# Lightbrite88/Argon_Monte_Carlo

Hardware: AMD Instinct MI355X
Metric: particle-steps/sec (higher is better)
Workload: dtype f64; 1 GPU; cube_1e5; geometry=cube, n_particles=100000, n_per_gpu=100000, parallelism=single GPU

## Files before the change

### argon_monte_carlo_amd/csrc/amc_api.hip

```cpp
#include <memory>
#include <type_traits>

#include "amc_host.h"

int amc_fail(amc_ctx *c, int code, const char *fmt, ...)
{
    char buf[512];
    va_list ap;
    va_start(ap, fmt);
    vsnprintf(buf, sizeof buf, fmt, ap);
    va_end(ap);
    if (c) c->err = buf;
    return code;
}

static thread_local std::string g_create_err;

void amc_prof_begin(amc_ctx *c, int kclass)
{
    if (!c->profiling) return;
    if (c->ev_used == c->ev_pool.size()) {
        hipEvent_t a, b;
        (void)ctx_event(c, &a, hipEventDefault);
        (void)ctx_event(c, &b, hipEventDefault);
// ... 95 lines not shown
    }
    if (off > 0x7fff0000LL) return amc_fail(c, AMC_ERR_INVALID, "detection grid too large (%lld cells)", off);
    G.ncells = (int)off;
    AMC_HIP(c, dalloc(c, &c->d_lay, (size_t)3 * G.gz));
    AMC_HIP(c, hipMemcpy(c->d_lay, c->h_lay_lo.data(), sizeof(int) * G.gz, hipMemcpyHostToDevice));
    AMC_HIP(c, hipMemcpy(c->d_lay + G.gz, c->h_lay_n.data(), sizeof(int) * G.gz, hipMemcpyHostToDevice));
    AMC_HIP(c, hipMemcpy(c->d_lay + 2 * G.gz, c->h_lay_off.data(), sizeof(int) * G.gz, hipMemcpyHostToDevice));
    G.lay_lo = c->d_lay; G.lay_n = c->d_lay + G.gz; G.lay_off = c->d_lay + 2 * G.gz;
    return AMC_OK;
}

static bool env_set(const char *name) { return getenv(name) != nullptr; }
static bool env_nonzero(const char *name) { const char *e = getenv(name); return e && atoi(e) != 0; }
static int env_int(const char *name, int unset) { const char *e = getenv(name); return e ? atoi(e) : unset; }
static long long env_ll(const char *name, long long unset) { const char *e = getenv(name); return e ? atoll(e) : unset; }

static void read_env(amc_ctx *c)
{
    const char *sync = getenv("AMC_OVERLAP_SYNC");
    c->ovl_sync_values = sync && !strcmp(sync, "value");
    c->overlap_mode = env_int("AMC_OVERLAP", 0);
    c->overlap_split = env_nonzero("AMC_OVERLAP_SPLIT");
    c->cw_blocks_env = env_int("AMC_CW_BLOCKS", 0);
    c->ordered_always = env_nonzero("AMC_ORDERED_ALWAYS");
    c->od_max_n = env_ll("AMC_OD_MAX_N", c->od_max_n);
    c->od_ahead = std::min(std::max(env_int("AMC_OD_AHEAD", c->od_ahead), 1), 32);
    if (const int v = env_int("AMC_PLAN_SMALL", -1); v >= 0) c->plan_small = v;
    c->stream_bs = env_int("AMC_STREAM_BS", 256);
    c->detect_bs = env_int("AMC_DETECT_BS", 256);
    c->temp_unfused = env_set("AMC_TEMP_UNFUSED");
    c->temp_run_unfused = !AMC_TEMP_RUN_FUSED_DEFAULT;
    if (env_nonzero("AMC_TEMP_RUN_FUSED")) c->temp_run_unfused = false;
    if (env_nonzero("AMC_TEMP_RUN_UNFUSED")) c->temp_run_unfused = true;
    c->allpairs_max_n = env_ll("AMC_ALLPAIRS_MAX_N", 0);
    const int g = c->P.geometry;
    c->list_keep = env_int("AMC_LIST_KEEP", (g == AMC_GEOM_PORE || g == AMC_GEOM_PORE_ENERGISED) ? AMC_LIST_KEEP_DEFAULT_PORE : 0);
    c->max_hist_env = env_int("AMC_MAX_HIST", 0);
    c->debug_resolve = env_set("AMC_DEBUG_RESOLVE");
}

static int alloc_state(amc_ctx *c)
{
    const size_t n = std::max<size_t>((size_t)c->n, 1);
    double **st[] = {&c->S.x, &c->S.y, &c->S.z, &c->S.vx, &c->S.vy, &c->S.vz, &c->S.d, &c->S.dx, &c->S.dy, &c->S.dz,
                     &c->S.px, &c->S.py, &c->S.pz};
    const size_t per = ((sizeof(double) * n) + 255) & ~(size_t)255;
// ... 451 lines not shown
        for (int v : h) { sum += v; top = std::max<int64_t>(top, v); }
    }
    out[0] = c->keep_K >= 2 ? c->keep_K : 0; out[1] = c->keep_K >= 2 ? c->B.wave_cap : 0; out[2] = (int64_t)waves;
    out[3] = cycle ? T.lists_age : -1; out[4] = owner; out[5] = sum; out[6] = top; out[7] = T.full_builds;
    return AMC_OK;
}

int amc_owned_count(amc_ctx *c, int64_t *count)
{
    if (!c || !count) return AMC_ERR_INVALID;
    *count = (int64_t)c->owned.size();
    return AMC_OK;
}

int amc_kernel_times(amc_ctx *c, double *total_ms, int64_t *launches)
{
    if (!c) return AMC_ERR_INVALID;
    hipSetDevice(c->device);
    amc_prof_collect(c);
    if (c->d_dbg) {
        long long h[128];
        hipMemcpy(h, c->d_dbg, sizeof h, hipMemcpyDeviceToHost);
        const double n = h[11] > 0 ? (double)h[11] : 1.0;
        fprintf(stderr, "[amc k_resolve phases, us/launch] count-left %.1f claim %.1f | rounds: collect %.1f pairs %.1f clusters>=3: sort+load %.1f emulate %.1f | overlay %.1f validate %.1f commit %.1f | rounds %.2f cand %.1f complex-members %.2f launches %lld (idle hand-over only %lld) | body: labels in the work space %lld moved there %lld layers in LDS %lld rounds split %lld heads shared %lld sorted %lld pool global %lld sort global %lld later %lld clusters by a wave %lld by one lane %lld most complex members %lld\n",
                h[0] / n / 100.0, h[1] / n / 100.0, h[6] / n / 100.0, h[7] / n / 100.0, h[2] / n / 100.0, h[3] / n / 100.0, h[14] / n / 100.0, h[4] / n / 100.0, h[5] / n / 100.0,
                h[8] / n, h[9] / n, h[10] / n, h[11], h[12], h[32], h[33], h[34], h[35], h[36], h[37], h[38], h[39], h[40], h[41], h[42], h[43]);
        fprintf(stderr, "[amc host candidate count] %d (what the next launch plan is chosen from)\n", c->h_host_ncand ? (int)*c->h_host_ncand : -1);
        if (h[12] > 0)
            fprintf(stderr, "[amc k_resolve idle hand-over, us/launch] entry -> counts read %.2f, -> hand-over written %.2f, -> through the barrier %.2f (%lld launches)\n",
                    h[16] / (double)h[12] / 100.0, h[17] / (double)h[12] / 100.0, h[18] / (double)h[12] / 100.0, h[12]);
        {
            std::vector<long long> wv((size_t)128 * 512);
            hipMemcpy(wv.data(), c->d_dbg + 128, sizeof(long long) * wv.size(), hipMemcpyDeviceToHost);
            long long s[128] = {0}, longest = 0;
            for (int w = 0; w < 512; w++) {
                for (int e = 3; e < 128; e++) if (e != 4) s[e] += wv[(size_t)128 * w + e];
                longest = std::max(longest, wv[(size_t)128 * w + 4]);
            }
            const double nl = h[25] > 0 ? (double)h[25] : 1.0;
            static const char *cn[8] = {"pair", "3-cluster", "4+-cluster", "not owner", "pair+again", "3-cluster+again", "4+-cluster+again", "not owner+again"};
            static const char *pn[12] = {"graph", "walk", "reserve", "small: after emulate", "pair emulate | by the wave: emulate", "publish", "grid probe", "first hop", "particles", "set-up", "overlay probe", "small: prepare"};
            fprintf(stderr, "[amc k_clusters_wide] working waves %lld in %lld launches; launch span (first working wave in -> last out) %.2f us, last out -> ordered workgroup in %.2f us, longest wave ever %.2f us\n",
                    s[3], h[25], h[27] / nl / 100.0, h[26] / nl / 100.0, longest / 100.0);
            fprintf(stderr, "[three-particle path of lane 0] %lld times, %lld continued from the pair's hit; loads + slots %.2f us, emulation %.2f us\n", s[5], s[6],
                    s[7] / (double)std::max<long long>(1, s[5]) / 100.0, s[124] / (double)std::max<long long>(1, s[5]) / 100.0);
            fprintf(stderr, "[pair-wave lifetimes, 2.5 us buckets]");
            for (int k = 0; k < 8; k++) fprintf(stderr, " %lld", s[24 + k]);
            fprintf(stderr, "\n");
            for (int k = 0; k < 8; k++) {
                if (!s[16 + k]) continue;
                fprintf(stderr, "[amc k_clusters_wide %-16s %7lld waves, %5.1f us]", cn[k], s[16 + k], s[8 + k] / (double)s[16 + k] / 100.0);
                for (int e = 0; e < 12; e++) fprintf(stderr, " %s %.2f", pn[e], s[32 + 12 * k + e] / (double)s[16 + k] / 100.0);
                fprintf(stderr, "\n");
            }
        }
    }
    for (int k = 0; k < AMC_K_COUNT; k++) {
        if (total_ms) total_ms[k] = c->k_ms[k];
        if (launches) launches[k] = c->k_launches[k];
    }
    return AMC_OK;
}

}
```

### argon_monte_carlo_amd/csrc/amc_clusters.hip

```cpp
#include <stdlib.h>

#define RS_WAVE_SYNC_LDS_ONLY 1
#include "amc_resolve_dev.h"

#define CW_MAXM 16
#define CW_MAXC 24
#define CW_ITEMS 192
#define CW_BLOCKS 512
#define CW_WPB 1

AMC_DEV int cw_adj_head(const amc_resolve_ws &W, unsigned int epoch, int p)
{
    const unsigned long long v = amc_g(W.adj_head)[p];
    return ((unsigned int)(v >> 32) == epoch) ? (int)(unsigned int)(v & 0xffffffffULL) : -1;
}

#define CW_ITERS 3
#define CW_PULLS 4

AMC_DEV void cw_init_slot(const amc_resolve_ws &W, int s, int p, int label, int gen, bool fresh = false)
{
    amc_g(W.slot_of)[p] = s; amc_g(W.sl_moved)[s] = 0;
    auto *m = amc_g((unsigned long long *)&W.sl_meta[s]);
    __hip_atomic_store(m + 0, ((unsigned long long)(unsigned int)label << 32) | (unsigned int)p, __ATOMIC_RELAXED, __HIP_MEMORY_SCOPE_AGENT);
// ... 5 lines not shown
{
    const auto *d = amc_g((const double *)&W.hist[h]);
    double4 r;
    r.x = __hip_atomic_load(d + 0, __ATOMIC_RELAXED, __HIP_MEMORY_SCOPE_AGENT);
    r.y = __hip_atomic_load(d + 1, __ATOMIC_RELAXED, __HIP_MEMORY_SCOPE_AGENT);
    r.z = __hip_atomic_load(d + 2, __ATOMIC_RELAXED, __HIP_MEMORY_SCOPE_AGENT);
    r.w = __hip_atomic_load(d + 3, __ATOMIC_RELAXED, __HIP_MEMORY_SCOPE_AGENT);
    return r;
}

struct cw_lds {
    int mem[64][CW_MAXM];
    int msl[64][CW_MAXM];
    int cnd[64][CW_MAXC];
    int pull[64][CW_PULLS], psl[64][CW_PULLS];
    int nm[64], nc[64], lab[64], npull[64];
    int it0[64];
    int used[64];
    int redo[64];
    int gen[64];
    cw_item item[CW_ITEMS];
    int next[CW_ITEMS];
    int nitems;
    int unv[64];
    double pool_d[10][CW_MAXM];
    int pool_tmp[CW_MAXM], pool_pidx[CW_MAXM], pool_slot[CW_MAXM];
    uint8_t pool_flag[CW_MAXM], pool_moved[CW_MAXM];
};

AMC_DEV void cw_probe_grid(const rs_args &A, rs_shared *wc, cw_lds &L, const cw_item &me, int cell, int s_off)
{
    const amc_resolve_ws &W = A.W;
    const int own = me.own, nm = L.nm[own], lab = L.lab[own];
    const double x = me.x, y = me.y, z = me.z;
    int q = amc_list_head(A.B, cell);
    while (q >= 0) {
        const amc_rec r = amc_g_load(&A.B.rec[q]);
        const int idx = amc_node_particle(A.B, q);
        q = amc_rec_next(r);
        double rx, ry, rz;
        amc_rec_pos(A.G, r, rx, ry, rz);
        const double ax = rx - x, ay = ry - y, az = rz - z;
        if (!(ax * ax + ay * ay + az * az < A.G.cr2_probe)) continue;
        bool mine = false;
        for (int m = 0; m < nm; m++) mine |= L.mem[own][m] == idx;
        if (mine) continue;
// ... 33 lines not shown
            if (t < 0 || t >= CW_ITEMS || L.item[t].h != h2) break;
            h2 = L.next[t];
        }
        return h2;
    };
    int h2 = skip_own(__hip_atomic_load(amc_g(W.ov_head) + cell, __ATOMIC_RELAXED, __HIP_MEMORY_SCOPE_AGENT));
    int guard = 0;
    while (h2 >= 0) {
        if (++guard > W.max_hist) { amc_g(wc)->ovf = 1; rs_raise(W); break; }
        const double4 o = cw_load_hist(W, h2);
        const int nx = __hip_atomic_load(amc_g(W.ov_next) + h2, __ATOMIC_RELAXED, __HIP_MEMORY_SCOPE_AGENT);
        h2 = skip_own(nx);
        const double ax = o.x - x, ay = o.y - y, az = o.z - z;
        if (!(ax * ax + ay * ay + az * az < cr2i)) continue;
        const int s2 = rs_hist_slot(o);
        bool mine = false;
        for (int m = 0; m < nm; m++) mine |= L.msl[own][m] == s2;
        if (mine) continue;
        if (rs_hist_gen(o) != __hip_atomic_load(amc_g((int *)&W.sl_meta[s2]) + 2, __ATOMIC_RELAXED, __HIP_MEMORY_SCOPE_AGENT)) continue;
        rs_add_edge(W, wc, me.p, -(s2 + 2));
    }
}

AMC_DEV int cw_prepare(const amc_resolve_ws &W, rs_shared *wc, cw_lds &L, int own, int h_off)
{
    int m = L.nm[own];
    const int lab = L.lab[own];
    const int np = L.npull[own] < CW_PULLS ? L.npull[own] : CW_PULLS;
    L.unv[own] = 0;
    for (int e = 0; e < np; e++) {
        const int v = L.pull[own][e], sv = L.psl[own][e];
        if (m == CW_MAXM) {
            cw_init_slot(W, sv, v, lab, 0);
            L.unv[own] = 2;
            continue;
        }
        int b = m - 1;
        while (b >= 0 && L.mem[own][b] > v) { L.mem[own][b + 1] = L.mem[own][b]; L.msl[own][b + 1] = L.msl[own][b]; b--; }
        L.mem[own][b + 1] = v; L.msl[own][b + 1] = sv;
        m++;
    }
    L.nm[own] = m; L.npull[own] = 0;
    L.used[own] = 0;
    L.it0[own] = -1;
    return m;
}
// ... 38 lines not shown
    int4 c4_first = make_int4(0, 0, -1, -1);
    unsigned long long mark_first = 0;
    if (lane < per && k_first < A_in_kernarg.W.max_cand) {
        c4_first = A_in_kernarg.W.cand4[k_first]; mark_first = A_in_kernarg.W.cand_mark[k_first];
    }
    int ncand = (int)__hip_atomic_load(&A_in_kernarg.O.cnt->cand_count, __ATOMIC_RELAXED, __HIP_MEMORY_SCOPE_AGENT);
    const int stalled = A_in_kernarg.od_stall ? *A_in_kernarg.od_stall : 0;
#pragma unroll
    for (int j = 0; j < ARG_TRIPS; j++) {
        const int i = (int)threadIdx.x + j * ARG_T;
        if (i < ARG_WORDS) ((int *)&s_args)[i] = arg_w[j];
    }
    __syncthreads();
    const rs_args &A = s_args;
    const amc_resolve_ws &W = A.W;
    rs_shared *wc = (rs_shared *)W.wctl;
    __shared__ cw_lds L_all[CW_WPB];
    cw_lds &L = L_all[threadIdx.x >> 6];
    if (stalled && A.od_tick > stalled) return;
    if (ncand > W.max_cand) ncand = W.max_cand;
    if (wave_id == 0 && lane == 0) {
        amc_g(wc)->active = 1; amc_g(wc)->ncand = ncand;
        if (A.od_done) *amc_g(A.od_done) = A.od_tick;
    }
    if (ncand == 0) return;
    const int s_off = 2 * ncand;
    const int h_off = 4 * ncand;
    const double cr2i = A.P.collision_range * A.P.collision_range * AMC_CR2_INFLATE;
    rs_work K;
    K.x = L.pool_d[0]; K.y = L.pool_d[1]; K.z = L.pool_d[2]; K.vx = L.pool_d[3]; K.vy = L.pool_d[4]; K.vz = L.pool_d[5];
    K.d = L.pool_d[6]; K.dx = L.pool_d[7]; K.dy = L.pool_d[8]; K.dz = L.pool_d[9];
    K.tmp = L.pool_tmp; K.pidx = L.pool_pidx; K.slot = L.pool_slot; K.flag = L.pool_flag; K.moved = L.pool_moved;

    long long t_last = t_enter__;
    long long t_acc[12] = {0, 0, 0, 0, 0, 0, 0, 0, 0, 0, 0, 0};
#define CW_STAMP(slot)                                                                     \
    do {                                                                                   \
        if (timed__) {                                                                     \
            const long long now__ = wall_clock64();                                        \
            t_acc[slot] += now__ - t_last;                                                 \
            t_last = now__;                                                                \
        }                                                                                  \
    } while (0)
    const bool timed__ = DBG && dbg__ && lane == 0 && wave_id * per < ncand;
    if (DBG && dbg__) { asm volatile("s_waitcnt vmcnt(0)" ::: "memory"); CW_STAMP(7); }
    int cat__ = 0;
    long long d_cont = 0, d_three = 0, d_t_load = 0, d_t_emu = 0;
    for (int k0 = wave_id * per; k0 < ncand; k0 += nwaves * per) {
        const int k = k0 + lane;
        const bool valid = lane < per && k < ncand;
        if (lane == 0) L.nitems = 0;
        int4 c4 = make_int4(0, 0, -1, -1);
        int head_i = -1, head_j = -1;
        amc_particle pre_j, pre_i;
        bool fh_ok = false;
        int fh_it0 = -1, fh_pj = -1, fh_pi = -1, fh_sj = -1, fh_si = -1;
        bool iso = false;
        int k2 = -1;
        int4 c4b = make_int4(0, 0, -1, -1);
        unsigned long long mkb = 0;
        if (valid) {
            c4 = (k == k_first) ? c4_first : amc_g_load(&W.cand4[k]);
            const unsigned long long mk = (k == k_first) ? mark_first : amc_g(W.cand_mark)[k];
            const bool marked = (unsigned int)(mk >> 32) == A.sweep_epoch;
            iso = c4.z < 0 && c4.w < 0 && !marked;
            if (c4.z < 0 && c4.w < 0 && marked) {
                const unsigned int succ = (unsigned int)(mk & 0xffffffffULL);
                if (succ != AMC_MARK_MULTI && (int)succ > k && (int)succ < ncand) k2 = (int)succ;
            }
            if (k2 >= 0) { c4b = amc_g_load(&W.cand4[k2]); mkb = amc_g(W.cand_mark)[k2]; }
// ... 172 lines not shown
                    for (int c = sub; c < 8; c += lpi) {
                        const int cell = amc_grid_box_cell<true>(A.G, it.x, it.y, it.z, A.G.cr_probe, c);
                        if (cell >= 0) cw_probe_grid(A, wc, L, it, cell, s_off);
                    }
                }
            }
            first_item = nit;
            CW_STAMP(6);
            if (!__ballot(L.redo[lane] != 0)) break;
            if (timed__ && L.redo[0]) cat__ |= 4;
            if (iter + 1 == CW_ITERS || L.nitems >= CW_ITEMS - 8) {
                if (L.redo[lane]) {
                    const int np = L.npull[lane] < CW_PULLS ? L.npull[lane] : CW_PULLS;
                    for (int e = 0; e < np; e++) cw_init_slot(W, L.psl[lane][e], L.pull[lane][e], L.lab[lane], 0);
                    rs_add_edge(W, wc, L.mem[lane][0], L.mem[lane][0]);
                    L.redo[lane] = 0;
                }
                break;
            }
        }
        rs_wave_sync();
        asm volatile("s_waitcnt vmcnt(0)" ::: "memory");
        const int nit = L.nitems < CW_ITEMS ? L.nitems : CW_ITEMS;
        for (int t0 = 0; t0 < nit; t0 += 64) {
            const int t = t0 + lane;
            if (t < nit) L.next[t] = -1;
            if (t < nit) {
                const cw_item it = L.item[t];
                if (!(it.pad & 1) && (it.pad >> 1) == L.gen[it.own]) {
                    int cx, cy, cz;
                    amc_grid_coords(A.G, it.x, it.y, it.z, cx, cy, cz);
                    const int cell = amc_grid_cell<true>(A.G, cx, cy, cz, nullptr);
                    int expected = -1;
                    for (;;) {
                        const int old = amc_atomic_cas(amc_g(W.ov_head) + cell, expected, it.h);
                        if (old == expected) break;
                        expected = old;
                        __hip_atomic_store(amc_g(W.ov_next) + it.h, old, __ATOMIC_RELAXED, __HIP_MEMORY_SCOPE_AGENT);
                        asm volatile("s_waitcnt vmcnt(0)" ::: "memory");
                    }
                    L.next[t] = expected;
                }
            }
        }
        asm volatile("s_waitcnt vmcnt(0)" ::: "memory");
        rs_wave_sync();
        CW_STAMP(5);
        {
            const int lpi = nit <= 8 ? 8 : (nit <= 16 ? 4 : (nit <= 32 ? 2 : 1));
            const int sub = lane % lpi;
            for (int t = lane / lpi; t < nit; t += 64 / lpi) {
                const cw_item it = L.item[t];
                if ((it.pad & 1) || (it.pad >> 1) != L.gen[it.own]) continue;
                for (int c = sub; c < 8; c += lpi) {
                    const int cell = amc_grid_box_cell<true>(A.G, it.x, it.y, it.z, A.G.cr_probe, c);
                    if (cell >= 0) cw_probe_overlay(A, wc, L, it, cell, cr2i, h_off);
                }
            }
        }
        rs_wave_sync();
        CW_STAMP(10);
    }
    if (timed__) {
        long long *R = dbg__ + 128 + 128 * (long long)wave_id;
        const long long t_exit = wall_clock64(), life = t_exit - t_enter__;
        R[0] = t_enter__; R[1] = t_exit; R[2] = A.sweep_epoch;
        R[3] += 1;
        if (life > R[4]) R[4] = life;
        R[5] += d_three; R[6] += d_cont; R[7] += d_t_load; R[124] += d_t_emu;
        R[8 + cat__] += life; R[16 + cat__] += 1;
        for (int e = 0; e < 12; e++) R[32 + 12 * cat__ + e] += t_acc[e];
        if (cat__ == 0) { int bk = (int)(life / 250); if (bk > 7) bk = 7; R[24 + bk] += 1; }
    }
}

int amc_clusters_wide_blocks(amc_ctx *c)
{
    const int nb_env = c->cw_blocks_env;
    if (nb_env > 0) return (nb_env + CW_WPB - 1) / CW_WPB * CW_WPB;
    return CW_BLOCKS;
}

hipError_t amc_launch_clusters_wide(amc_ctx *c, const rs_args &A)
{
    const int nb = amc_clusters_wide_blocks(c);
    const dim3 grid((nb + CW_WPB - 1) / CW_WPB), block(64 * CW_WPB);
    const bool cube = c->P.geometry == AMC_GEOM_CUBE;
    if (A.dbg) {
        if (cube) AMC_LAUNCH(c, (k_clusters_wide<AMC_GEOM_CUBE, true>), grid, block, A);
        else AMC_LAUNCH(c, (k_clusters_wide<AMC_GEOM_PORE, true>), grid, block, A);
    } else {
        if (cube) AMC_LAUNCH(c, (k_clusters_wide<AMC_GEOM_CUBE, false>), grid, block, A);
// ... 5 lines not shown
```

### argon_monte_carlo_amd/csrc/amc_grid.hip

```cpp
#include <stdlib.h>

#include "amc_grid_dev.h"

#define AMC_CR2_INFLATE (1.0 + 1.0e-9)

__global__ __launch_bounds__(256) void k_bin_lists(const double *__restrict__ x, const double *__restrict__ y,
                                                   const double *__restrict__ z, long long n, amc_grid G, amc_lists B,
                                                   amc_dev_counters *cnt, amc_ovl V)
{
    const long long p = (long long)blockIdx.x * blockDim.x + threadIdx.x;
    if (p >= n) return;
    if (V.skip_epoch && (unsigned int)(V.adj_head[p] >> 32) == V.skip_epoch) return;
    bool outside = false;
    amc_list_insert(G, B, (int)p, x[p], y[p], z[p], &outside);
    if (outside) atomicOr(&cnt->flags, 8ULL);
}

struct amc_adj {
    unsigned long long *head;
    int4 *rec;
    int4 *sd;
    int4 *sl_meta;
    int *sl_hits, *ev_gen;
    unsigned int epoch;
    unsigned long long *mark;
};

AMC_DEV int amc_push_candidate(int a, int b, int max_cand, amc_dev_counters *cnt, const amc_adj &D)
{
    const unsigned int k = atomicAdd(&cnt->cand_count, 1u);
    if (k < (unsigned)max_cand) {
        const int hi = a > b ? a : b, lo = a > b ? b : a;
        int4 r;
        r.x = hi; r.y = lo; r.z = -1; r.w = -1;
        if (D.head) {
            const unsigned long long mine = ((unsigned long long)D.epoch << 32) | (unsigned long long)k;
            const unsigned long long oi = atomicExch(&D.head[hi], mine), oj = atomicExch(&D.head[lo], mine);
            r.z = ((unsigned int)(oi >> 32) == D.epoch) ? (int)(unsigned int)(oi & 0xffffffffULL) : -1;
            r.w = ((unsigned int)(oj >> 32) == D.epoch) ? (int)(unsigned int)(oj & 0xffffffffULL) : -1;
            auto mark = [&](int kd) {
                const unsigned long long old = atomicExch(&D.mark[kd], mine);
                if ((unsigned int)(old >> 32) == D.epoch) D.mark[kd] = ((unsigned long long)D.epoch << 32) | AMC_MARK_MULTI;
            };
            if (r.z >= 0) mark(r.z);
            if (r.w >= 0) mark(r.w);
        }
        D.rec[k] = r;
        D.sd[k] = make_int4(-1, -1, 0, 0);
        if (D.head) {
            D.sl_meta[2 * k] = make_int4(-1, 2 * (int)k, 0, 0);
            D.sl_meta[2 * k + 1] = make_int4(-1, 2 * (int)k + 1, 0, 0);
            atomicAnd(&D.sl_hits[2 * k], 0);
            atomicAnd(&D.sl_hits[2 * k + 1], 0);
            *(int4 *)&D.ev_gen[4 * k] = make_int4(0, 0, 0, 0);
        }
        return (int)k;
    }
    atomicOr(&cnt->flags, 1ULL);
    return -1;
}

AMC_DEV void amc_detect_node(const amc_grid &G, const amc_lists &B, int node, double cr2i, double cr_probe, int max_cand,
                             amc_dev_counters *cnt, const amc_adj &D, const int *od_stall = nullptr, int od_tick = 0)
{
    const int stalled = od_stall ? *od_stall : 0;
    amc_rec me_r = B.rec[node];
    const int live = (B.node_of && node < B.n) ? B.node_of[node] : node;
    if (stalled && od_tick > stalled) return;
    if (me_r.x != me_r.x) {
        if (live == node) return;
        node = live;
        me_r = B.rec[node];
        if (me_r.x != me_r.x) return;
    }
    const int me_p = amc_node_particle(B, node);
    double3 me;
    amc_rec_pos(G, me_r, me.x, me.y, me.z);
// ... 250 lines not shown
                for (int r = 0; r < AP2_R; r++)
                    if (fma(az[r], jz, fma(ay[r], jy, fma(ax[r], jx, jn))) < ti[r] && (diag ? j < ii[r] : true))
                        amc_push_candidate(ii[r], j, max_cand, cnt, D);
            }
        }
    }
}

static unsigned int next_sweep_epoch(unsigned int epoch)
{
    epoch = (epoch + 1u) & 0x3fffffffu;
    return epoch ? epoch : 1u;
}

hipError_t amc_launch_detect(amc_ctx *c)
{
    const long long n = c->n;
    if (n <= 0) return hipSuccess;
    const double cr2i = c->allpairs || c->detect_ap ? c->P.collision_range * c->P.collision_range * AMC_CR2_INFLATE : c->G.cr2_probe;
    amc_adj D;
    c->step.sweep_epoch = next_sweep_epoch(c->step.sweep_epoch);
    c->step.plan_split = !c->allpairs && !(c->h_host_ncand && *c->h_host_ncand <= c->plan_small);
    D.head = c->allpairs ? nullptr : c->W.adj_head; D.rec = c->W.cand4; D.sd = c->W.cand_s; D.epoch = c->step.sweep_epoch;
    D.sl_meta = c->W.sl_meta; D.sl_hits = c->W.sl_hits; D.ev_gen = c->W.ev_gen; D.mark = c->W.cand_mark;
    amc_prof_begin(c, AMC_K_DETECT);
    if (c->detect_ap) {
        if (n >= 16 * AP2_T && c->G.ncells > 0) {
            const int ntiles = (int)((n + AP2_T - 1) / AP2_T);
            const long long nblocks = (long long)ntiles * (ntiles + 1) / 2;
            const double ex = c->G.gx * c->G.h, ey = c->G.gy * c->G.h, ez = c->G.gz * c->G.h;
            const double thr = cr2i + 64.0 * 1.1102230246251565e-16 * (ex * ex + ey * ey + ez * ez);
            AMC_LAUNCH(c, k_detect_allpairs_tiled, dim3((unsigned)nblocks), dim3(AP2_THREADS), c->S.x, c->S.y,
                               c->S.z, (int)n, ntiles, thr, c->G.x0, c->G.y0, c->G.z0, c->W.max_cand, c->d_cnt, D);
        } else {
            const int ntiles = (int)((n + AP_T - 1) / AP_T);
            const long long nblocks = (long long)ntiles * (ntiles + 1) / 2;
            if (nblocks > 0)
                AMC_LAUNCH(c, k_detect_allpairs, dim3((unsigned)nblocks), dim3(AP_T), c->S.x, c->S.y,
                                   c->S.z, (int)n, ntiles, cr2i, c->W.max_cand, c->d_cnt, D);
        }
    } else {
        const bool extras = c->B.extra != nullptr && c->keep_K < 2;
        const int slot = (c->B.extra == c->extra_buf[1]) ? 1 : 0;
        const int bs = c->detect_bs;
        AMC_LAUNCH(c, k_detect_lists, dim3((unsigned)((n + bs - 1) / bs) + (extras ? 4u : 0u)), dim3(bs), c->G, c->B, n, cr2i,
                   c->G.cr_probe, c->W.max_cand, c->d_cnt, D, (const int *)(extras ? c->extra_count + slot : nullptr),
                   c->max_extra, (const int *)(c->od_active ? c->d_od : nullptr), c->od_tick,
                   (c->od_active && !c->step.od_prev_ordered) ? c->W.wctl : nullptr);
    }
    amc_prof_end(c);
    return hipGetLastError();
}

hipError_t amc_launch_detect_own(amc_ctx *c)
{
    const long long cnt = c->hi - c->lo;
    amc_prof_begin(c, AMC_K_DETECT);
    if (cnt > 0)
        AMC_LAUNCH(c, k_detect_own, dim3((unsigned)((cnt + 255) / 256)), dim3(256), c->G, c->B, (long long)c->lo, (long long)c->hi,
                   c->G.cr2_probe, c->G.cr_probe, c->MG.cand_send, c->MG.cand_cap, c->d_cnt);
    amc_prof_end(c);
    return hipGetLastError();
}

hipError_t amc_launch_ingest(amc_ctx *c, int world)
{
    amc_adj D;
    c->step.sweep_epoch = next_sweep_epoch(c->step.sweep_epoch);
    c->step.plan_split = !(c->h_host_ncand && *c->h_host_ncand <= c->plan_small);
    D.head = c->W.adj_head; D.rec = c->W.cand4; D.sd = c->W.cand_s; D.epoch = c->step.sweep_epoch;
    D.sl_meta = c->W.sl_meta; D.sl_hits = c->W.sl_hits; D.ev_gen = c->W.ev_gen; D.mark = c->W.cand_mark;
    amc_prof_begin(c, AMC_K_DETECT);
    AMC_LAUNCH(c, k_ingest_candidates, dim3(16), dim3(256), (const int *)c->MG.cand_recv, world, 2 + 2 * c->MG.cand_cap, c->MG.cand_cap,
               c->W.max_cand, c->d_cnt, D, c->MG.cand_send);
    amc_prof_end(c);
    return hipGetLastError();
}
```

### argon_monte_carlo_amd/csrc/amc_internal.h

```cpp
#pragma once
#include <hip/hip_runtime.h>
#include <hip/hip_ext.h>
#include <stdint.h>

#include <string>
#include <vector>

#include "amc_device.h"

#define RS_SLOT_DOUBLES 12

struct amc_state {
    double *x, *y, *z, *vx, *vy, *vz, *d, *dx, *dy, *dz;
    double *px, *py, *pz;
    uint8_t *flag;
};

struct amc_grid {
    double x0, y0, z0, h;
    double inv_h;
    int uniform;
    int gx, gy, gz;
    int ncells;
    double cr_probe;
// ... 251 lines not shown
    int kin_world;
    int64_t kin_m, kin_cap, kin_block;
    int *cand_send, *cand_recv;
    int cand_cap, cand_world;
    int *wave_count;
    int waves_pack, waves_unpack;
    bool keep;
    long long *hits_send, *hits_recv;
    int *hits_perm;
    int hits_cap, hits_view_world;
    int hits_tile;
    int64_t hits_rows;
    amc_mg_step step;
};

enum amc_res_kind { AMC_RES_DEVICE, AMC_RES_PINNED, AMC_RES_STREAM, AMC_RES_EVENT };
struct amc_res { void *p; amc_res_kind kind; };

#define AMC_OD_AHEAD 2
#define AMC_OD_MAX_N 100000
#define AMC_OD_RING 64
#define AMC_OD_MIN_STEPS 8
#define AMC_PLAN_SMALL 430

struct amc_step_state {
    bool lazy_pending;
    bool commit_pending;
    bool commit_defer;
    int commit_step = 0;
    unsigned int sweep_epoch;
    bool plan_split;
    int lists_age = -1;
    int lists_owner;
    bool od_prev_ordered = true;
    int64_t full_builds = 0;
};

struct amc_ctx {
    amc_params P;
    int device;
    hipStream_t own_stream, stream;
    std::string err;
    int64_t n, lo, hi;
    bool uploaded;
    bool keep_prior;
    std::vector<amc_res> owned;
// ... 17 lines not shown
    amc_temp_dev_ws TD;
    amc_wall_law wall_law = {};
    amc_moments_ws F;
    amc_surface_ws SF;
    amc_corr_ws CR;
    amc_moments_ws FX;
    amc_mfp_ws MF;
    amc_vdf_ws VD;
    amc_transit_ws TR;
    amc_pair_ws PD;
    amc_out out;
    amc_path_record *d_rec;
    unsigned long long *d_hist;
    double *d_edges;
    amc_dev_counters *d_cnt;
    amc_counter_bank *d_banks;
    amc_dev_counters h_prev;
    long long *d_dbg;
    char *h_pin;
    size_t h_pin_bytes;
    int overlap_mode;
    bool overlap_split;
    int cw_blocks_env;
    int stream_bs;
    int detect_bs;
    bool temp_unfused;
    bool temp_run_unfused;
    bool ordered_always;
    int64_t od_max_n = AMC_OD_MAX_N;
    int od_ahead = AMC_OD_AHEAD;
    int plan_small = AMC_PLAN_SMALL;
    long long allpairs_max_n;
    int list_keep;
    int max_hist_env;
    bool debug_resolve;
    bool profiling;
    double k_ms[AMC_K_COUNT];
    int64_t k_launches[AMC_K_COUNT];
    std::vector<std::pair<hipEvent_t, hipEvent_t>> ev_pool;
    std::vector<std::pair<int, int>> ev_pending;
    size_t ev_used;
    hipEvent_t prof_ev0, prof_ev1;
    amc_state S_buf[2];
    char *s_slab2;
    amc_lists B_buf[2];
    int *extra_buf[2];
// ... 96 lines not shown
```

### argon_monte_carlo_amd/csrc/amc_resolve.hip

```cpp
#include <stdlib.h>
#include <algorithm>

#include "amc_resolve_dev.h"
#include "amc_commit_dev.h"

#define RS_STAMP(slot)                                                                     \
    do {                                                                                   \
        if (A.dbg && tid == 0) {                                                           \
            const long long now__ = wall_clock64();                                        \
            A.dbg[slot] += now__ - t_last;                                                 \
            t_last = now__;                                                                \
        }                                                                                  \
    } while (0)

#define RS_NS 6144
#define RS_LAY 4096

template <int GEOM, int MODE>
__global__ __launch_bounds__(RS_T) void k_resolve(rs_args A_in_kernarg)
{
    const rs_args &K = A_in_kernarg;
    long long t_last = (K.dbg && threadIdx.x == 0) ? wall_clock64() : 0;
    if (K.dbg && MODE == 0 && K.wide_plan) {
        const rs_args &A = K;
// ... 334 lines not shown
                const amc_particle q = rs_load_particle(A.S, p);
                rs_store_work(K, w, q);
                K.moved[w] = 0;
                K.pidx[w] = p;
                K.slot[w] = W.slot_of[p];
            }
            __syncthreads();
            for (int w = tid; w < nc; w += RS_T) {
                const unsigned lab = (unsigned)(keys[w] >> 32);
                if (w > 0 && (unsigned)(keys[w - 1] >> 32) == lab) continue;
                int e = w + 1;
                while (e < nc && (unsigned)(keys[e] >> 32) == lab) e++;
                if (A.dbg && e - w >= 2) atomicAdd((unsigned long long *)&A.dbg[42], 1ULL);
                if (e - w >= 2) rs_emulate_generic(A, &sh, K, w, e);
            }
            __syncthreads();
            for (int w = tid; w < nc; w += RS_T)
                if (K.moved[w]) rs_store_slot(W, K.slot[w], rs_load_work(K, w));
        }
        __syncthreads();
        RS_STAMP(3);
        const int nh = sh.nhist < W.max_hist ? sh.nhist : W.max_hist;
        if (!A.allpairs) {
            for (int h = sh.hist_begin + tid; h < nh; h += RS_T) W.ov_next[h] = atomicExch(&W.ov_head[rs_hist_cell(A, G, h)], h);
            __syncthreads();
            if (A.dbg && tid == 0) { const long long n__ = wall_clock64(); A.dbg[14] += n__ - t_last; }
            for (int h = sh.hist_begin + tid; h < nh; h += RS_T) rs_probe(A, G, &sh, V.label, ns, V.cap, h, cr2i);
        } else {
            const int hb = sh.hist_begin;
            for (long long w = tid; w < (long long)(nh - hb) * A.n; w += RS_T) {
                const int h = hb + (int)(w / A.n);
                const int idx = (int)(w % A.n);
                const double4 hr = W.hist[h];
                if (rs_hist_gen(hr) == 0) continue;
                const int sme = rs_hist_slot(hr);
                if (idx == W.sl_meta[sme].x) continue;
                const double ex = A.S.x[idx] - hr.x, ey = A.S.y[idx] - hr.y, ez = A.S.z[idx] - hr.z;
                if (ex * ex + ey * ey + ez * ez < cr2i) {
                    const int so = W.slot_of[idx];
                    if (so >= 0 && so < ns && V.label[so] == V.label[sme]) continue;
                    if (so < 0) rs_claim_slot(W, &sh, V.cap, idx);
                    rs_add_edge(W, &sh, W.sl_meta[sme].x, idx);
                }
            }
            for (long long w = tid; w < (long long)(nh - hb) * nh; w += RS_T) {
                const int h = hb + (int)(w / nh), h2 = (int)(w % nh);
// ... 87 lines not shown
                rs_apply_slot(W, A.S, s, p);
            }
            W.slot_of[p] = -1;
        }
        return;
    }
    amc_commit_args C;
    C.ctl = (amc_resolve_ctl *)W.ctl; C.hist = W.hist; C.ov_head = W.ov_head; C.ev_gen = W.ev_gen; C.ev = W.ev;
    C.sl_meta = W.sl_meta; C.sl_hits = W.sl_hits; C.sl_moved = W.sl_moved; C.sl_state = W.sl_state; C.slot_of = W.slot_of;
    C.max_slots = W.max_slots; C.max_hist = W.max_hist; C.lo = A.lo; C.hi = A.hi; C.count_pp = A.count_pp;
    C.defer = A.defer_commit; C.nogrid = A.allpairs; C.enabled = 1; C.step = A.O.step;
    C.od_stall = nullptr; C.od_tick = 0; C.from_wide = 0; C.wctl = nullptr; C.host_ncand = nullptr;
    amc_commit_part(C, A.O, A.G, A.S, gtid, gstride);
}

static int rs_wide_per(amc_ctx *c)
{
    const long long lag = c->h_host_ncand ? *c->h_host_ncand : 0;
    const long long nb = amc_clusters_wide_blocks(c);
    const long long per = (lag + lag / 4 + nb - 1) / nb;
    return (int)std::min<long long>(std::max<long long>(per, 1), 64);
}

template <int GEOM>
static void rs_launch_all(amc_ctx *c, const rs_args &A)
{
    if (c->allpairs) {
        AMC_LAUNCH(c, (k_resolve<GEOM, 2>), dim3(1), dim3(RS_T), A);
        return;
    }
    rs_args Aw = A;
    Aw.wide_plan = 1;
    Aw.force_mono = 0;
    Aw.wide_per = rs_wide_per(c);
    amc_prof_cancel(c);
    amc_prof_begin(c, AMC_K_CLUSTERS_WIDE);
    amc_launch_clusters_wide(c, Aw);
    amc_prof_end(c);
    amc_prof_begin(c, AMC_K_RESOLVE);
    AMC_LAUNCH(c, (k_resolve<GEOM, 0>), dim3(1), dim3(RS_T), Aw);
    c->od_ordered_launches++;
    c->step.od_prev_ordered = true;
    c->step.commit_defer = A.defer_commit != 0;
    if (A.defer_commit) { c->step.commit_pending = true; c->step.commit_step = c->out.step; return; }
    amc_prof_end(c);
    amc_prof_begin(c, AMC_K_COMMIT);
    AMC_LAUNCH(c, k_commit, dim3(AMC_COMMIT_BLOCKS), dim3(256), Aw);
}

static rs_args rs_make_args(amc_ctx *c)
{
    rs_args A;
    A.P.collision_range = c->P.collision_range; A.P.argon_mass = c->P.argon_mass; A.P.dx = c->P.dx; A.P.dy = c->P.dy; A.P.dz = c->P.dz;
    A.P.overlap_x = c->P.overlap_x; A.P.overlap_y = c->P.overlap_y; A.P.overlap_z = c->P.overlap_z;
    A.P.nx = c->P.nx; A.P.ny = c->P.ny; A.P.nz = c->P.nz; A.P.geometry = c->P.geometry;
    A.S = c->S; A.G = c->G; A.B = c->B; A.W = c->W; A.O = c->out; A.n = c->n; A.allpairs = c->allpairs ? 1 : 0;
    A.dbg = c->d_dbg;
    A.force_mono = 0;
    A.host_ncand = c->d_host_ncand;
    A.plan_small = c->plan_small;
    A.defer_commit = 0;
    A.apply_only = 0;
    A.sweep_epoch = c->step.sweep_epoch;
    A.wide_plan = 0;
    A.count_pp = c->MG.count_pp ? 1 : 0;
    A.lo = c->lo; A.hi = c->hi;
    A.inv_dx = c->P.dx > 0 ? 1.0 / c->P.dx : 0.0; A.inv_dy = c->P.dy > 0 ? 1.0 / c->P.dy : 0.0; A.inv_dz = c->P.dz > 0 ? 1.0 / c->P.dz : 0.0;
    A.W.raise_dev = nullptr; A.W.raise_host = nullptr; A.W.raise_tick = 0;
    A.od_stall = nullptr; A.od_stall_host = nullptr; A.od_done = nullptr; A.od_tick = 0;
    return A;
}

hipError_t amc_launch_wide_only(amc_ctx *c, rs_args *used)
{
    rs_args Aw = rs_make_args(c);
    Aw.defer_commit = 1;
    Aw.wide_plan = 1;
    Aw.wide_per = rs_wide_per(c);
    Aw.W.raise_dev = c->d_od; Aw.W.raise_host = c->d_od_stall_host; Aw.W.raise_tick = c->od_tick;
    Aw.od_stall = c->d_od; Aw.od_stall_host = c->d_od_stall_host; Aw.od_done = c->d_od_done_host; Aw.od_tick = c->od_tick;
    amc_prof_begin(c, AMC_K_CLUSTERS_WIDE);
    amc_launch_clusters_wide(c, Aw);
    amc_prof_end(c);
    c->step.commit_defer = true;
    c->step.commit_pending = true;
    c->step.commit_step = c->out.step;
    c->step.od_prev_ordered = false;
    c->od_steps++;
    *used = Aw;
    return hipGetLastError();
}

hipError_t amc_launch_ordered(amc_ctx *c, const rs_args &used)
{
    rs_args Aw = used;
    Aw.W.raise_dev = nullptr; Aw.W.raise_host = nullptr;
    Aw.od_done = nullptr;
    amc_prof_begin(c, AMC_K_RESOLVE);
    if (c->P.geometry == AMC_GEOM_CUBE) AMC_LAUNCH(c, (k_resolve<AMC_GEOM_CUBE, 0>), dim3(1), dim3(RS_T), Aw);
    else AMC_LAUNCH(c, (k_resolve<AMC_GEOM_PORE, 0>), dim3(1), dim3(RS_T), Aw);
    amc_prof_end(c);
// ... 38 lines not shown
```

### argon_monte_carlo_amd/csrc/amc_resolve_dev.h

```cpp
#pragma once
#include "amc_grid_dev.h"

#define RS_T 512
#define RS_SORT_LDS 2048
#define RS_POOL 256
#define RS_MAX_ROUNDS 256
#define AMC_CR2_INFLATE (1.0 + 1.0e-9)

#ifdef RS_WAVE_SYNC_LDS_ONLY
#define RS_CNT(p) amc_g(p)
#else
#define RS_CNT(p) (p)
#endif

struct rs_geom {
    double collision_range, argon_mass, dx, dy, dz, overlap_x, overlap_y, overlap_z;
    int nx, ny, nz, geometry;
};

struct rs_args {
    rs_geom P;
    amc_state S;
    amc_lists B;
    amc_grid G;
    amc_resolve_ws W;
    amc_out O;
    long long n;
    int allpairs;
    int defer_commit;
    int apply_only;
    int force_mono;
    int plan_small;
    int *host_ncand;
    int count_pp;
    long long lo, hi;
    double inv_dx, inv_dy, inv_dz;
    long long *dbg;
    unsigned int sweep_epoch;
    int wide_plan;
    int wide_per;
    int *od_stall, *od_stall_host, *od_done;
    int od_tick;
};


struct amc_ctx;
hipError_t amc_launch_clusters_wide(amc_ctx *c, const rs_args &A);
int amc_clusters_wide_blocks(amc_ctx *c);

struct rs_shared {
    int nslots, nedges, nhist, nev, dirty, changed, nhits, nfp, ovf, nclusters, ncomplex;
    int rounds, ncand, active, ok, edges_done;
    int lazy_ns;
    int nslots0;
    int hist_begin;
    int cur_round;
};

AMC_DEV void rs_raise(const amc_resolve_ws &W)
{
    if (W.raise_dev) { *amc_g(W.raise_dev) = W.raise_tick; *amc_g(W.raise_host) = W.raise_tick; }
}

struct rs_work {
    double *x, *y, *z, *vx, *vy, *vz, *d, *dx, *dy, *dz;
// ... 770 lines not shown
```

Before: 2.394 billion particle-steps/s.

## Add dense all-vs-history scan for small candidate counts in wide cluster kernel

When the candidate count is at most a threshold (default 256, capped by wide blocks × per-wave), the wide cluster kernel skips the per-cell overlay linking. Each wave instead checks its items against every history entry in a register-blocked dense scan. The resolve kernel links all valid history entries into the overlay on its first wide round, and the detect path clears the hist w field so slot reuse is correct. This trades grid-probe and linked-list traversal for brute-force distance tests, which helps when the candidate count is small and costs more when it is large.

```diff
diff --git a/argon_monte_carlo_amd/csrc/amc_api.hip b/argon_monte_carlo_amd/csrc/amc_api.hip
--- a/argon_monte_carlo_amd/csrc/amc_api.hip
+++ b/argon_monte_carlo_amd/csrc/amc_api.hip
@@ -141,6 +141,7 @@
     c->overlap_mode = env_int("AMC_OVERLAP", 0);
     c->overlap_split = env_nonzero("AMC_OVERLAP_SPLIT");
     c->cw_blocks_env = env_int("AMC_CW_BLOCKS", 0);
+    c->cw_dense_max = std::max(env_int("AMC_CW_DENSE_MAX", c->cw_dense_max), 0);
     c->ordered_always = env_nonzero("AMC_ORDERED_ALWAYS");
     c->od_max_n = env_ll("AMC_OD_MAX_N", c->od_max_n);
     c->od_ahead = std::min(std::max(env_int("AMC_OD_AHEAD", c->od_ahead), 1), 32);
@@ -638,9 +639,9 @@
         long long h[128];
         hipMemcpy(h, c->d_dbg, sizeof h, hipMemcpyDeviceToHost);
         const double n = h[11] > 0 ? (double)h[11] : 1.0;
-        fprintf(stderr, "[amc k_resolve phases, us/launch] count-left %.1f claim %.1f | rounds: collect %.1f pairs %.1f clusters>=3: sort+load %.1f emulate %.1f | overlay %.1f validate %.1f commit %.1f | rounds %.2f cand %.1f complex-members %.2f launches %lld (idle hand-over only %lld) | body: labels in the work space %lld moved there %lld layers in LDS %lld rounds split %lld heads shared %lld sorted %lld pool global %lld sort global %lld later %lld clusters by a wave %lld by one lane %lld most complex members %lld\n",
+        fprintf(stderr, "[amc k_resolve phases, us/launch] count-left %.1f claim %.1f | rounds: collect %.1f pairs %.1f clusters>=3: sort+load %.1f emulate %.1f | overlay %.1f validate %.1f commit %.1f | rounds %.2f cand %.1f complex-members %.2f launches %lld (idle hand-over only %lld) | body: labels in the work space %lld moved there %lld layers in LDS %lld rounds split %lld heads shared %lld sorted %lld pool global %lld sort global %lld later %lld clusters by a wave %lld by one lane %lld most complex members %lld dense sweeps linked %lld\n",
                 h[0] / n / 100.0, h[1] / n / 100.0, h[6] / n / 100.0, h[7] / n / 100.0, h[2] / n / 100.0, h[3] / n / 100.0, h[14] / n / 100.0, h[4] / n / 100.0, h[5] / n / 100.0,
-                h[8] / n, h[9] / n, h[10] / n, h[11], h[12], h[32], h[33], h[34], h[35], h[36], h[37], h[38], h[39], h[40], h[41], h[42], h[43]);
+                h[8] / n, h[9] / n, h[10] / n, h[11], h[12], h[32], h[33], h[34], h[35], h[36], h[37], h[38], h[39], h[40], h[41], h[42], h[43], h[44]);
         fprintf(stderr, "[amc host candidate count] %d (what the next launch plan is chosen from)\n", c->h_host_ncand ? (int)*c->h_host_ncand : -1);
         if (h[12] > 0)
             fprintf(stderr, "[amc k_resolve idle hand-over, us/launch] entry -> counts read %.2f, -> hand-over written %.2f, -> through the barrier %.2f (%lld launches)\n",
@@ -656,8 +657,8 @@
             const double nl = h[25] > 0 ? (double)h[25] : 1.0;
             static const char *cn[8] = {"pair", "3-cluster", "4+-cluster", "not owner", "pair+again", "3-cluster+again", "4+-cluster+again", "not owner+again"};
             static const char *pn[12] = {"graph", "walk", "reserve", "small: after emulate", "pair emulate | by the wave: emulate", "publish", "grid probe", "first hop", "particles", "set-up", "overlay probe", "small: prepare"};
-            fprintf(stderr, "[amc k_clusters_wide] working waves %lld in %lld launches; launch span (first working wave in -> last out) %.2f us, last out -> ordered workgroup in %.2f us, longest wave ever %.2f us\n",
-                    s[3], h[25], h[27] / nl / 100.0, h[26] / nl / 100.0, longest / 100.0);
+            fprintf(stderr, "[amc k_clusters_wide] working waves %lld in %lld launches; launch span (first working wave in -> last out) %.2f us, last out -> ordered workgroup in %.2f us, longest wave ever %.2f us; dense scans %lld\n",
+                    s[3], h[25], h[27] / nl / 100.0, h[26] / nl / 100.0, longest / 100.0, s[125]);
             fprintf(stderr, "[three-particle path of lane 0] %lld times, %lld continued from the pair's hit; loads + slots %.2f us, emulation %.2f us\n", s[5], s[6],
                     s[7] / (double)std::max<long long>(1, s[5]) / 100.0, s[124] / (double)std::max<long long>(1, s[5]) / 100.0);
             fprintf(stderr, "[pair-wave lifetimes, 2.5 us buckets]");
diff --git a/argon_monte_carlo_amd/csrc/amc_clusters.hip b/argon_monte_carlo_amd/csrc/amc_clusters.hip
--- a/argon_monte_carlo_amd/csrc/amc_clusters.hip
+++ b/argon_monte_carlo_amd/csrc/amc_clusters.hip
@@ -51,6 +51,7 @@
     cw_item item[CW_ITEMS];
     int next[CW_ITEMS];
     int nitems;
+    int ncand;
     int unv[64];
     double pool_d[10][CW_MAXM];
     int pool_tmp[CW_MAXM], pool_pidx[CW_MAXM], pool_slot[CW_MAXM];
@@ -130,6 +131,74 @@
     }
 }
 
+#define CW_DENSE_U 8
+AMC_DEV void cw_dense_hit(const amc_resolve_ws &W, rs_shared *wc, cw_lds &L, int own, int p, int s2, int g2)
+{
+    const int nm = L.nm[own];
+    if ((unsigned int)s2 >= (unsigned int)W.max_slots) return;
+    bool mine = false;
+    for (int m = 0; m < nm; m++) mine |= L.msl[own][m] == s2;
+    if (mine || g2 != __hip_atomic_load(amc_g((int *)&W.sl_meta[s2]) + 2, __ATOMIC_RELAXED, __HIP_MEMORY_SCOPE_AGENT)) return;
+    rs_add_edge(W, wc, p, -(s2 + 2));
+}
+AMC_DEV void cw_scan_dense(const amc_resolve_ws &W, rs_shared *wc, cw_lds &L, int nit_in, int ncand, double cr2i, int lane)
+{
+    const int npair = 2 * ncand;
+    const int nit = __builtin_amdgcn_readfirstlane(nit_in);
+    if (nit == 0) return;
+    for (int base = 0; base < npair; base += 64 * CW_DENSE_U) {
+        double4 o[CW_DENSE_U];
+        double w2[CW_DENSE_U];
+        int gen[CW_DENSE_U];
+        unsigned int second = 0;
+#pragma unroll
+        for (int u = 0; u < CW_DENSE_U; u++) {
+            const int i = base + 64 * u + lane, ic = min(i, npair - 1), h = 4 * (ic >> 1) + (ic & 1);
+            o[u] = cw_load_hist(W, h);
+            w2[u] = __hip_atomic_load(amc_g((const double *)&W.hist[h + 2]) + 3, __ATOMIC_RELAXED, __HIP_MEMORY_SCOPE_AGENT);
+        }
+#pragma unroll
+        for (int u = 0; u < CW_DENSE_U; u++) {
+            const int in = (base + 64 * u + lane - npair) >> 31;
+            gen[u] = rs_hist_gen(o[u]) & in;
+            second |= ((int)(__double_as_longlong(w2[u]) >> 32) & in) != 0 ? 1u << u : 0u;
+        }
+        for (int t = 0; t < nit; t++) {
+            const int pad = __builtin_amdgcn_readfirstlane(L.item[t].pad), own = __builtin_amdgcn_readfirstlane(L.item[t].own);
+            if ((pad & 1) || (pad >> 1) != __builtin_amdgcn_readfirstlane(L.gen[own])) continue;
+            const double x = L.item[t].x, y = L.item[t].y, z = L.item[t].z;
+            const int kc = __builtin_amdgcn_readfirstlane(L.cnd[own][0]);
+            unsigned int hits = 0;
+#pragma unroll
+            for (int u = 0; u < CW_DENSE_U; u++) {
+                const double ax = o[u].x - x, ay = o[u].y - y, az = o[u].z - z;
+                const bool pass = (ax * ax + ay * ay + az * az < cr2i) & (gen[u] != 0) & (((base + 64 * u + lane) >> 1) != kc);
+                hits |= pass ? 1u << u : 0u;
+            }
+            while (hits) {
+                const int u = __ffs((int)hits) - 1;
+                hits &= hits - 1;
+                int s2 = 0, g2 = 0;
+#pragma unroll
+                for (int e = 0; e < CW_DENSE_U; e++) { s2 = (e == u) ? rs_hist_slot(o[e]) : s2; g2 = (e == u) ? gen[e] : g2; }
+                cw_dense_hit(W, wc, L, own, L.item[t].p, s2, g2);
+            }
+        }
+        while (second) {
+            const int u = __ffs((int)second) - 1;
+            second &= second - 1;
+            const int i = base + 64 * u + lane;
+            const double4 o2 = cw_load_hist(W, 4 * (i >> 1) + (i & 1) + 2);
+            for (int t = 0; t < nit; t++) {
+                const cw_item me = L.item[t];
+                if ((me.pad & 1) || (me.pad >> 1) != L.gen[me.own]) continue;
+                const double ax = o2.x - me.x, ay = o2.y - me.y, az = o2.z - me.z;
+                if (rs_hist_gen(o2) != 0 && ax * ax + ay * ay + az * az < cr2i) cw_dense_hit(W, wc, L, me.own, me.p, rs_hist_slot(o2), rs_hist_gen(o2));
+            }
+        }
+    }
+}
+
 AMC_DEV int cw_prepare(const amc_resolve_ws &W, rs_shared *wc, cw_lds &L, int own, int h_off)
 {
     int m = L.nm[own];
@@ -214,11 +283,15 @@
     if (wave_id == 0 && lane == 0) {
         amc_g(wc)->active = 1; amc_g(wc)->ncand = ncand;
         if (A.od_done) *amc_g(A.od_done) = A.od_tick;
+        if (ncand <= A.dense_max && ncand > nwaves * per) { amc_g(wc)->ovf = 1; rs_raise(W); }
     }
     if (ncand == 0) return;
     const int s_off = 2 * ncand;
     const int h_off = 4 * ncand;
     const double cr2i = A.P.collision_range * A.P.collision_range * AMC_CR2_INFLATE;
+#define CW_DENSE(n) (__builtin_amdgcn_readfirstlane((n) <= A.dense_max) != 0)
+    L.ncand = ncand;
+    if (lane == 0) L.nitems = 0;
     rs_work K;
     K.x = L.pool_d[0]; K.y = L.pool_d[1]; K.z = L.pool_d[2]; K.vx = L.pool_d[3]; K.vy = L.pool_d[4]; K.vz = L.pool_d[5];
     K.d = L.pool_d[6]; K.dx = L.pool_d[7]; K.dy = L.pool_d[8]; K.dz = L.pool_d[9];
@@ -238,6 +311,7 @@
     if (DBG && dbg__) { asm volatile("s_waitcnt vmcnt(0)" ::: "memory"); CW_STAMP(7); }
     int cat__ = 0;
     long long d_cont = 0, d_three = 0, d_t_load = 0, d_t_emu = 0;
+    long long d_dense = 0;
     for (int k0 = wave_id * per; k0 < ncand; k0 += nwaves * per) {
         const int k = k0 + lane;
         const bool valid = lane < per && k < ncand;
@@ -456,6 +530,7 @@
         rs_wave_sync();
         asm volatile("s_waitcnt vmcnt(0)" ::: "memory");
         const int nit = L.nitems < CW_ITEMS ? L.nitems : CW_ITEMS;
+        if (CW_DENSE(ncand)) break;
         for (int t0 = 0; t0 < nit; t0 += 64) {
             const int t = t0 + lane;
             if (t < nit) L.next[t] = -1;
@@ -495,13 +570,24 @@
         rs_wave_sync();
         CW_STAMP(10);
     }
+    asm volatile("" ::: "memory");
+    if (CW_DENSE(L.ncand)) {
+        const int nit = L.nitems < CW_ITEMS ? L.nitems : CW_ITEMS;
+        CW_STAMP(5);
+        if (DBG) d_dense = 1;
+        const int lane_again = (int)__builtin_amdgcn_mbcnt_hi(~0u, __builtin_amdgcn_mbcnt_lo(~0u, 0u));
+        const double cr = A.P.collision_range;
+        cw_scan_dense(W, (rs_shared *)W.wctl, L, nit, L.ncand, cr * cr * AMC_CR2_INFLATE, lane_again);
+        rs_wave_sync();
+        CW_STAMP(10);
+    }
     if (timed__) {
         long long *R = dbg__ + 128 + 128 * (long long)wave_id;
         const long long t_exit = wall_clock64(), life = t_exit - t_enter__;
         R[0] = t_enter__; R[1] = t_exit; R[2] = A.sweep_epoch;
         R[3] += 1;
         if (life > R[4]) R[4] = life;
-        R[5] += d_three; R[6] += d_cont; R[7] += d_t_load; R[124] += d_t_emu;
+        R[5] += d_three; R[6] += d_cont; R[7] += d_t_load; R[124] += d_t_emu; R[125] += d_dense;
         R[8 + cat__] += life; R[16 + cat__] += 1;
         for (int e = 0; e < 12; e++) R[32 + 12 * cat__ + e] += t_acc[e];
         if (cat__ == 0) { int bk = (int)(life / 250); if (bk > 7) bk = 7; R[24 + bk] += 1; }
diff --git a/argon_monte_carlo_amd/csrc/amc_grid.hip b/argon_monte_carlo_amd/csrc/amc_grid.hip
--- a/argon_monte_carlo_amd/csrc/amc_grid.hip
+++ b/argon_monte_carlo_amd/csrc/amc_grid.hip
@@ -22,6 +22,7 @@
     int4 *sd;
     int4 *sl_meta;
     int *sl_hits, *ev_gen;
+    double4 *hist;
     unsigned int epoch;
     unsigned long long *mark;
 };
@@ -53,6 +54,8 @@
             atomicAnd(&D.sl_hits[2 * k], 0);
             atomicAnd(&D.sl_hits[2 * k + 1], 0);
             *(int4 *)&D.ev_gen[4 * k] = make_int4(0, 0, 0, 0);
+#pragma unroll
+            for (int e = 0; e < 4; e++) D.hist[4 * k + e].w = 0.0;
         }
         return (int)k;
     }
@@ -349,7 +352,7 @@
     c->step.sweep_epoch = next_sweep_epoch(c->step.sweep_epoch);
     c->step.plan_split = !c->allpairs && !(c->h_host_ncand && *c->h_host_ncand <= c->plan_small);
     D.head = c->allpairs ? nullptr : c->W.adj_head; D.rec = c->W.cand4; D.sd = c->W.cand_s; D.epoch = c->step.sweep_epoch;
-    D.sl_meta = c->W.sl_meta; D.sl_hits = c->W.sl_hits; D.ev_gen = c->W.ev_gen; D.mark = c->W.cand_mark;
+    D.sl_meta = c->W.sl_meta; D.sl_hits = c->W.sl_hits; D.ev_gen = c->W.ev_gen; D.mark = c->W.cand_mark; D.hist = c->W.hist;
     amc_prof_begin(c, AMC_K_DETECT);
     if (c->detect_ap) {
         if (n >= 16 * AP2_T && c->G.ncells > 0) {
@@ -396,7 +399,7 @@
     c->step.sweep_epoch = next_sweep_epoch(c->step.sweep_epoch);
     c->step.plan_split = !(c->h_host_ncand && *c->h_host_ncand <= c->plan_small);
     D.head = c->W.adj_head; D.rec = c->W.cand4; D.sd = c->W.cand_s; D.epoch = c->step.sweep_epoch;
-    D.sl_meta = c->W.sl_meta; D.sl_hits = c->W.sl_hits; D.ev_gen = c->W.ev_gen; D.mark = c->W.cand_mark;
+    D.sl_meta = c->W.sl_meta; D.sl_hits = c->W.sl_hits; D.ev_gen = c->W.ev_gen; D.mark = c->W.cand_mark; D.hist = c->W.hist;
     amc_prof_begin(c, AMC_K_DETECT);
     AMC_LAUNCH(c, k_ingest_candidates, dim3(16), dim3(256), (const int *)c->MG.cand_recv, world, 2 + 2 * c->MG.cand_cap, c->MG.cand_cap,
                c->W.max_cand, c->d_cnt, D, c->MG.cand_send);
diff --git a/argon_monte_carlo_amd/csrc/amc_internal.h b/argon_monte_carlo_amd/csrc/amc_internal.h
--- a/argon_monte_carlo_amd/csrc/amc_internal.h
+++ b/argon_monte_carlo_amd/csrc/amc_internal.h
@@ -297,6 +297,7 @@
 #define AMC_OD_RING 64
 #define AMC_OD_MIN_STEPS 8
 #define AMC_PLAN_SMALL 430
+#define AMC_CW_DENSE_MAX 256
 
 struct amc_step_state {
     bool lazy_pending;
@@ -360,6 +361,7 @@
     int overlap_mode;
     bool overlap_split;
     int cw_blocks_env;
+    int cw_dense_max = AMC_CW_DENSE_MAX;
     int stream_bs;
     int detect_bs;
     bool temp_unfused;
diff --git a/argon_monte_carlo_amd/csrc/amc_resolve.hip b/argon_monte_carlo_amd/csrc/amc_resolve.hip
--- a/argon_monte_carlo_amd/csrc/amc_resolve.hip
+++ b/argon_monte_carlo_amd/csrc/amc_resolve.hip
@@ -380,6 +380,15 @@
         RS_STAMP(3);
         const int nh = sh.nhist < W.max_hist ? sh.nhist : W.max_hist;
         if (!A.allpairs) {
+            if (first && wide && ncand <= A.dense_max) {
+                if (A.dbg && tid == 0) A.dbg[44] += 1;
+                for (int h = tid; h < wide_nh; h += RS_T) {
+                    const double4 r = W.hist[h];
+                    const int g = rs_hist_gen(r), s = rs_hist_slot(r);
+                    if (g == 0 || s < 0 || s >= W.max_slots || g != W.sl_meta[s].z) continue;
+                    W.ov_next[h] = atomicExch(&W.ov_head[rs_hist_cell(A, G, h)], h);
+                }
+            }
             for (int h = sh.hist_begin + tid; h < nh; h += RS_T) W.ov_next[h] = atomicExch(&W.ov_head[rs_hist_cell(A, G, h)], h);
             __syncthreads();
             if (A.dbg && tid == 0) { const long long n__ = wall_clock64(); A.dbg[14] += n__ - t_last; }
@@ -513,6 +522,11 @@
     return (int)std::min<long long>(std::max<long long>(per, 1), 64);
 }
 
+static int rs_dense_max(amc_ctx *c, int wide_per)
+{
+    return (int)std::min<long long>(c->cw_dense_max, (long long)amc_clusters_wide_blocks(c) * wide_per);
+}
+
 template <int GEOM>
 static void rs_launch_all(amc_ctx *c, const rs_args &A)
 {
@@ -524,6 +538,7 @@
     Aw.wide_plan = 1;
     Aw.force_mono = 0;
     Aw.wide_per = rs_wide_per(c);
+    Aw.dense_max = rs_dense_max(c, Aw.wide_per);
     amc_prof_cancel(c);
     amc_prof_begin(c, AMC_K_CLUSTERS_WIDE);
     amc_launch_clusters_wide(c, Aw);
@@ -559,6 +574,7 @@
     A.inv_dx = c->P.dx > 0 ? 1.0 / c->P.dx : 0.0; A.inv_dy = c->P.dy > 0 ? 1.0 / c->P.dy : 0.0; A.inv_dz = c->P.dz > 0 ? 1.0 / c->P.dz : 0.0;
     A.W.raise_dev = nullptr; A.W.raise_host = nullptr; A.W.raise_tick = 0;
     A.od_stall = nullptr; A.od_stall_host = nullptr; A.od_done = nullptr; A.od_tick = 0;
+    A.dense_max = 0;
     return A;
 }
 
@@ -568,6 +584,7 @@
     Aw.defer_commit = 1;
     Aw.wide_plan = 1;
     Aw.wide_per = rs_wide_per(c);
+    Aw.dense_max = rs_dense_max(c, Aw.wide_per);
     Aw.W.raise_dev = c->d_od; Aw.W.raise_host = c->d_od_stall_host; Aw.W.raise_tick = c->od_tick;
     Aw.od_stall = c->d_od; Aw.od_stall_host = c->d_od_stall_host; Aw.od_done = c->d_od_done_host; Aw.od_tick = c->od_tick;
     amc_prof_begin(c, AMC_K_CLUSTERS_WIDE);
diff --git a/argon_monte_carlo_amd/csrc/amc_resolve_dev.h b/argon_monte_carlo_amd/csrc/amc_resolve_dev.h
--- a/argon_monte_carlo_amd/csrc/amc_resolve_dev.h
+++ b/argon_monte_carlo_amd/csrc/amc_resolve_dev.h
@@ -41,6 +41,7 @@
     int wide_per;
     int *od_stall, *od_stall_host, *od_done;
     int od_tick;
+    int dense_max;
 };
 
 
```

Result: faster. 2.425 billion particle-steps/s, median of 6 (+1.3%).
